# microscopic-image-analysis/geosss

Measured on AMD Instinct MI355X. Metric: mcmc_chain_steps_per_sec, higher is better.
Workload: dtype f64; 1 GPU; vmfmix_readme: shrinkage slice sampler, 1000000 chains/GPU x 1000 transitions per launch, thin=100; target=vmfmix_readme, d=3, chains_per_gpu=1000000, thin=100, mode=fast, kernel=screened_kernel<3, ScreenVmf<3, 3>>, kept_rows_layout=components, slice_steps=500, library_matches_tree=True, stream=philox-v3 (chain,step)-keyed; S2: tangent = one angle; 32-bit tries

## Files before the change

geosss_amd/csrc/gsss_device.h:

```cpp
#pragma once
#include <hip/hip_runtime.h>
#include <stdint.h>
#include <stdlib.h>

#include <algorithm>
#include <vector>

#include "../../include/gsss.h"
#include "gsss_counter_words.h"
#include "gsss_math.h"

namespace gsss {

constexpr int kBlock = 256;
constexpr double kTwoPi = 6.283185307179586;

struct TargetBlock {
    const double *blob;
    int32_t kind, d, k, dpad;
    double kappa;
    double scale;
};

struct RunBlock {
// ... 521 lines not shown
        hop = s[(size_t)r.r_hop * n];
        psum = s[(size_t)r.r_p * n];
        psq = s[(size_t)(r.r_p + 1) * n];
        pos = r.L > 0 ? (int)(cnt % (int64_t)r.L) : 0;
#pragma unroll
        for (int l = 0; l < kStatsMaxLags; ++l) {
            const bool in = l < r.L;
            lag[l] = in ? s[(size_t)(r.r_lag + (in ? l : 0)) * n] : 0.0;
            if (in) ring[(size_t)l * kBlock] = s[(size_t)(r.r_ring + l) * n];
        }
    }

    __device__ __forceinline__ void draw(const RunBlock &a, int64_t c, const double (&x)[D])
    {
        const size_t n = (size_t)a.n_chains;
        double *s = a.stats + c;
        const Rows r = rows(a);
        const double *w = a.stats_dirs, *h = a.stats_dirs + D, *modes = a.stats_dirs + 2 * D;
        double p = 0.0, xh = 0.0;
#pragma unroll
        for (int j = 0; j < D; ++j) {
            p = fma(x[j], w[j], p);
            xh = fma(x[j], h[j], xh);
        }
        if (cnt > 0) {
            double dot = 0.0, ph = 0.0;
#pragma unroll
            for (int j = 0; j < D; ++j) {
                dot = fma(prev[j], x[j], dot);
                ph = fma(prev[j], h[j], ph);
            }
            dist += acos(fmin(fmax(dot, -1.0), 1.0));
            const int sa = (xh > 0.0) - (xh < 0.0), sb = (ph > 0.0) - (ph < 0.0);
            if (sa != sb) hop += 1.0;
        }
        int t = 0;
#pragma unroll
        for (int i = 0; i < D; ++i) {
            prev[i] = x[i];
            sum[i] += x[i];
            if (r.second) {
#pragma unroll
                for (int j = i; j < D; ++j) {
                    if (kXXRegs)
                        xx[t] += x[i] * x[j];
                    else
                        s[(size_t)(r.r_xx + t) * n] += x[i] * x[j];
                    ++t;
                }
            }
        }
        if (r.K > 0) {
            int best = 0;
            double bv = -INFINITY;
            for (int k = 0; k < r.K; ++k) {
                double v = 0.0;
#pragma unroll
                for (int j = 0; j < D; ++j) v = fma(x[j], modes[k * D + j], v);
                if (v > bv) {
                    bv = v;
                    best = k;
                }
            }
            s[(size_t)(r.r_mode + best) * n] += 1.0;
        }
        psum += p;
        psq += p * p;
        if (r.L > 0) {
            const int lm = cnt < (int64_t)r.L ? (int)cnt : r.L;
            int si = pos;
#pragma unroll
            for (int l = 1; l <= kStatsMaxLags; ++l) {
                si = si == 0 ? r.L - 1 : si - 1;
                if (l <= lm) lag[l - 1] += p * ring[(size_t)si * kBlock];
            }
            ring[(size_t)pos * kBlock] = p;
            if (cnt < r.L) s[(size_t)(r.r_head + cnt) * n] = p;
            pos = pos + 1 == r.L ? 0 : pos + 1;
        }
        ++cnt;
    }

    __device__ __forceinline__ void store(const RunBlock &a, int64_t c)
    {
        const size_t n = (size_t)a.n_chains;
        double *s = a.stats + c;
        const Rows r = rows(a);
        s[0] = (double)cnt;
#pragma unroll
        for (int i = 0; i < D; ++i) {
            s[(size_t)(r.r_prev + i) * n] = prev[i];
            s[(size_t)(r.r_sum + i) * n] = sum[i];
        }
        if (kXXRegs && r.second) {
#pragma unroll
            for (int t = 0; t < kT; ++t) s[(size_t)(r.r_xx + t) * n] = xx[t];
        }
        s[(size_t)r.r_dist * n] = dist;
        s[(size_t)r.r_hop * n] = hop;
        s[(size_t)r.r_p * n] = psum;
        s[(size_t)(r.r_p + 1) * n] = psq;
#pragma unroll
        for (int l = 0; l < kStatsMaxLags; ++l) {
            if (l < r.L) {
                s[(size_t)(r.r_lag + l) * n] = lag[l];
                s[(size_t)(r.r_ring + l) * n] = ring[(size_t)l * kBlock];
            }
        }
    }
};

__device__ __forceinline__ void philox4x32_10(uint32_t c0, uint32_t c1, uint32_t c2, uint32_t c3, uint32_t k0,
                                              uint32_t k1, uint32_t (&o)[4])
{
    k0 = (uint32_t)__builtin_amdgcn_readfirstlane((int)k0);
    k1 = (uint32_t)__builtin_amdgcn_readfirstlane((int)k1);
    asm volatile("" : "+s"(k0), "+s"(k1));
#pragma unroll
    for (int r = 0; r < 10; ++r) {
        const uint64_t p0 = (uint64_t)0xD2511F53u * c0;
        const uint64_t p1 = (uint64_t)0xCD9E8D57u * c2;
        const uint32_t n0 = __builtin_amdgcn_bitop3_b32((uint32_t)(p1 >> 32), c1, k0, 0x96);
        const uint32_t n2 = __builtin_amdgcn_bitop3_b32((uint32_t)(p0 >> 32), c3, k1, 0x96);
        c1 = (uint32_t)p1;
        c3 = (uint32_t)p0;
        c0 = n0;
        c2 = n2;
        k0 += 0x9E3779B9u;
        k1 += 0xBB67AE85u;
    }
    o[0] = c0; o[1] = c1; o[2] = c2; o[3] = c3;
}

__device__ __forceinline__ double try_uniform(uint32_t w) { return (double)w * 0x1.0p-32; }

__device__ __forceinline__ double u53(uint32_t a, uint32_t b)
{
    return fma((double)(a >> 5), 67108864.0, (double)(b >> 6)) * 0x1.0p-53;
}

__device__ __forceinline__ void box_muller32(uint32_t wr, uint32_t wa, double &z0, double &z1)
{
    float f0, f1;
    fm::box_muller_f32(wr, wa, f0, f1);
    z0 = (double)f0;
    z1 = (double)f1;
}

__device__ __forceinline__ void box_muller32(uint32_t wr, uint32_t wa, const fm::Tables &, double &z0, double &z1)
{
    box_muller32(wr, wa, z0, z1);
}

__device__ __forceinline__ void tangent3(double n0, double n1, double n2, double sn, double cs, double &u0, double &u1, double &u2)
{
    const double s = copysign(1.0, n2);
    const double a = -1.0 / (s + n2);
    const double b = n0 * n1 * a;
    const double b10 = 1.0 + s * n0 * n0 * a, b11 = s * b, b12 = -s * n0;
    const double b20 = b, b21 = s + n1 * n1 * a, b22 = -n1;
    u0 = fma(sn, b20, cs * b10);
    u1 = fma(sn, b21, cs * b11);
    u2 = fma(sn, b22, cs * b12);
}

constexpr int kTabLds = 2 * 64 + 2;
__device__ __forceinline__ fm::Tables stage_tables(double *lds_after_params)
{
    double *buf = lds_after_params + ((reinterpret_cast<uintptr_t>(lds_after_params) >> 3) & 1u);
    for (int i = threadIdx.x; i < 64; i += kBlock) fm::table_entry(buf, i);
    return fm::Tables{buf, nullptr};
}

constexpr uint64_t kInitStep = 0xFFFFFFFFFFFFull;

template <int D_>
struct LaneVec {
    static constexpr int L = 1;
    static constexpr int N = D_;
    static constexpr int DPAD = D_;
    static constexpr bool kExactDim = true;
    __device__ static __forceinline__ int comp(int , int i) { return i; }
    __device__ static __forceinline__ double reduce(double v) { return v; }
};

constexpr int kDppXor1 = 0xB1;
constexpr int kDppXor2 = 0x4E;
constexpr int kDppHalfMirror = 0x141;
constexpr int kDppMirror = 0x140;

template <int CTRL>
__device__ __forceinline__ double dpp_move(double v)
{
    const int lo = __builtin_amdgcn_update_dpp(0, __double2loint(v), CTRL, 0xF, 0xF, true);
    const int hi = __builtin_amdgcn_update_dpp(0, __double2hiint(v), CTRL, 0xF, 0xF, true);
    return __hiloint2double(hi, lo);
}
template <int CTRL>
__device__ __forceinline__ int dpp_move(int v)
{
    return __builtin_amdgcn_update_dpp(0, v, CTRL, 0xF, 0xF, true);
}
__device__ __forceinline__ double lane_broadcast(double v, int lane)
{
    const int lo = __builtin_amdgcn_readlane(__double2loint(v), lane);
    const int hi = __builtin_amdgcn_readlane(__double2hiint(v), lane);
    return __hiloint2double(hi, lo);
}

template <int L_>
__device__ __forceinline__ double group_sum(double v)
{
    if (L_ >= 2) v += dpp_move<kDppXor1>(v);
    if (L_ >= 4) v += dpp_move<kDppXor2>(v);
    if (L_ >= 8) v += dpp_move<kDppHalfMirror>(v);
    if (L_ >= 16) v += dpp_move<kDppMirror>(v);
    if (L_ == 64) {
        const double r0 = lane_broadcast(v, 0), r1 = lane_broadcast(v, 16);
        const double r2 = lane_broadcast(v, 32), r3 = lane_broadcast(v, 48);
        v = (r0 + r1) + (r2 + r3);
    }
    return v;
}

template <int L_, int S_>
struct CoopVec {
    static_assert(S_ % 4 == 0, "slots come in quads");
    static constexpr int L = L_;
    static constexpr int N = S_;
    static constexpr int DPAD = L_ * S_;
    static constexpr bool kExactDim = false;
    __device__ static __forceinline__ int comp(int g, int i) { return 4 * (g + L_ * (i >> 2)) + (i & 3); }
    static_assert(L_ == 2 || L_ == 4 || L_ == 8 || L_ == 16 || L_ == 64, "group sizes with a DPP reduction");
    __device__ static __forceinline__ double reduce(double v) { return group_sum<L_>(v); }
};

template <class V>
__device__ __forceinline__ double vdot(const double (&a)[V::N], const double (&b)[V::N])
{
    double s = 0.0;
#pragma unroll
    for (int i = 0; i < V::N; ++i) s = fma(a[i], b[i], s);
    return V::reduce(s);
}

template <class V>
__device__ __forceinline__ void stats_update_group(const RunBlock &a, int64_t c, int g, int d, const double (&x)[V::N])
{
    constexpr int N = V::N, LG = V::L;
    const size_t n = (size_t)a.n_chains;
    double *s = a.stats + c;
    const int K = a.stats_modes, L = a.stats_lags;
    const bool second = !(a.stats_flags & GSSS_STATS_NO_SECOND_MOMENT);
    const int T = second ? d * (d + 1) / 2 : 0;
    const int r_prev = 1, r_sum = 1 + d, r_xx = 1 + 2 * d, r_dist = r_xx + T, r_hop = r_dist + 1, r_mode = r_hop + 1;
    const int r_p = r_mode + K, r_lag = r_p + 2, r_ring = r_lag + L, r_head = r_ring + L;
    const double *w = a.stats_dirs, *h = a.stats_dirs + d, *modes = a.stats_dirs + 2 * d;
    const int64_t cnt = (int64_t)V::reduce(g == 0 ? s[0] : 0.0);
    double p = 0.0, xh = 0.0, dot = 0.0, ph = 0.0;
#pragma unroll
    for (int i = 0; i < N; ++i) {
        const int cc = V::comp(g, i);
        if (cc < d) {
            p = fma(x[i], w[cc], p);
            xh = fma(x[i], h[cc], xh);
            if (cnt > 0) {
                const double pj = s[(size_t)(r_prev + cc) * n];
                dot = fma(pj, x[i], dot);
                ph = fma(pj, h[cc], ph);
            }
        }
    }
    p = V::reduce(p);
    xh = V::reduce(xh);
    dot = V::reduce(dot);
    ph = V::reduce(ph);
    if (cnt > 0 && g == 0) {
        s[(size_t)r_dist * n] += acos(fmin(fmax(dot, -1.0), 1.0));
        const int sa = (xh > 0.0) - (xh < 0.0), sb = (ph > 0.0) - (ph < 0.0);
        if (sa != sb) s[(size_t)r_hop * n] += 1.0;
    }
#pragma unroll
    for (int i = 0; i < N; ++i) {
        const int cc = V::comp(g, i);
        if (cc < d) {
            s[(size_t)(r_prev + cc) * n] = x[i];
            s[(size_t)(r_sum + cc) * n] += x[i];
        }
    }
    if (second) {
        const int base = (int)(threadIdx.x % 64) - g;
        for (int jl = 0; jl < LG; ++jl) {
#pragma unroll
            for (int j = 0; j < N; ++j) {
                const double xj = __shfl(x[j], base + jl);
                const int cj = V::comp(jl, j);
#pragma unroll
                for (int i = 0; i < N; ++i) {
                    const int ci = V::comp(g, i);
                    if (cj < d && ci <= cj) s[(size_t)(r_xx + ci * d - ci * (ci - 1) / 2 + (cj - ci)) * n] += x[i] * xj;
                }
            }
        }
    }
    if (K > 0) {
        int best = 0;
        double bv = -INFINITY;
        for (int k = 0; k < K; ++k) {
            double v = 0.0;
#pragma unroll
// ... 1106 lines not shown
```

geosss_amd/csrc/gsss_screen.h:

```cpp
#pragma once
#include <type_traits>

#include "gsss_fast.h"
#include "gsss_screen_consts.h"

namespace gsss {

enum : int32_t { kFinalAccept = 3, kFinalDecide = 4, kFinalInHi = 2 };
__device__ __forceinline__ bool is_final(int32_t st) { return st >= kFinalAccept; }
__device__ __forceinline__ bool is_decide(int32_t st) { return st == kFinalDecide || st == kFinalDecide + kFinalInHi; }

__device__ __forceinline__ void sincos_rev32(double theta, float &s, float &c)
{
    const float t = (float)(theta * 0.15915494309189535);
    s = __builtin_amdgcn_sinf(t);
    c = __builtin_amdgcn_cosf(t);
}

__device__ __forceinline__ float log2_32(double v)
{
    int e;
    const double m = frexp(v, &e);
    return (float)e + __builtin_amdgcn_logf((float)m);
}

template <int D, int KC>
struct ScreenVmf : FastVmf<D, KC> {
    using Base = FastVmf<D, KC>;
    using Coef = typename Base::Coef;
    static constexpr int kCoef32Floats = 3 * KC + 1;
    static constexpr int kParkSkip = KC >= 6 ? 2 * KC : 0;
    static constexpr int kMinWaves = D > 10 ? ((D <= 12 && KC <= 3) ? 3 : 2) : (KC >= 6 ? 3 : ((D == 3 && KC <= 3) ? 5 : 1));
    static constexpr int kTradeMin = KC >= 6 ? 24 : 1;
    static constexpr int kSharedMinWaves = kMinWaves;
    static constexpr bool kCompact = false;
    static constexpr bool kOneAhead = KC == 10 || (KC == 6 && D <= 8) || (KC == 16 && D <= 5) || (KC == 4 && D == 3) || (KC == 3 && D == 4);
    static constexpr bool kStageRows = kOneAhead;
    static constexpr bool kHoldRows = false;
    static constexpr bool kPreferOne = kOneAhead;
    static constexpr int kNumpyWaves = (KC >= 10 || (D >= 9 && KC >= 6)) ? 2 : ((D <= 4 && KC <= 3) ? 4 : 3);
    static constexpr bool kRegenThr = D == 3 && KC <= 3;
    static constexpr bool kLog2Rows = D == 3 && KC <= 3;
    static_assert(!kLog2Rows || kParkSkip == 0, "refill() would have to form its floats from the scaled rows too");
    __host__ __device__ static constexpr size_t log2_doubles() { return kLog2Rows ? (size_t)KC * D + KC : 0; }
    __device__ void stage_log2(double *lds, const TargetBlock &tb)
    {
        constexpr double L = 1.4426950408889634074;
        Base::stage(lds, tb);
        __syncthreads();
        const int rows = (int)Base::lds_doubles();
        for (int i = threadIdx.x; i < rows; i += kBlock) lds[rows + i] = lds[i] * L;
    }
    __device__ __forceinline__ static void dots(const double *rows, int k, const double (&x)[D], const double (&u)[D], double &ax, double &au)
    {
        ax = 0.0, au = 0.0;
#pragma unroll
        for (int j = 0; j < D; ++j) {
            const double mkj = rows[k * D + j];
            ax = fma(mkj, x[j], ax);
            au = fma(mkj, u[j], au);
        }
    }
    __device__ __forceinline__ void retail(float (&)[kCoef32Floats]) const {}
    __device__ __forceinline__ void refill(const double (&x)[D], const double (&u)[D], float (&q)[kCoef32Floats]) const
    {
        constexpr double L = 1.4426950408889634074;
#pragma unroll
        for (int k = 0; k < KC; ++k) {
            double ax = 0.0, au = 0.0;
#pragma unroll
            for (int j = 0; j < D; ++j) {
                const double mkj = this->mu[k * D + j];
                ax = fma(mkj, x[j], ax);
                au = fma(mkj, u[j], au);
            }
            q[k] = (float)(ax * L);
            q[KC + k] = (float)(au * L);
        }
    }

    __device__ __forceinline__ void coeffs(Coef &cf, const double (&x)[D], const double (&u)[D]) const
    {
#pragma unroll
        for (int k = 0; k < KC; ++k) dots(this->mu, k, x, u, cf.ax[k], cf.au[k]);
        double m = -INFINITY;
#pragma unroll
        for (int k = 0; k < KC; ++k) m = fmax(m, cf.ax[k] + this->logc[k]);
        cf.m = m;
    }
    __device__ __forceinline__ bool make32(const Coef &cf, double u_thr, float (&q)[kCoef32Floats]) const
    {
        constexpr double L = 1.4426950408889634074;
        float s0 = 0.0f;
#pragma unroll
        for (int k = 0; k < KC; ++k) {
            q[k] = (float)(cf.ax[k] * L);
            q[KC + k] = (float)(cf.au[k] * L);
            q[2 * KC + k] = (float)((this->logc[k] - cf.m) * L);
            s0 += __builtin_amdgcn_exp2f(q[k] + q[2 * KC + k]);
        }
        return finish32(u_thr, q, s0);
    }
    __device__ __forceinline__ bool finish32(double u_thr, float (&q)[kCoef32Floats], float s0) const
    {
        float b = 0.0f;
        int e;
        const float m0 = frexpf(s0, &e);
        const float t2 = ((float)e + __builtin_amdgcn_logf(m0)) + log2_32(u_thr);
#pragma unroll
        for (int k = 0; k < KC; ++k) {
            q[2 * KC + k] -= t2;
            if (k < this->K) b = fmaxf(b, fabsf(q[k]) + fabsf(q[KC + k]) + fabsf(q[2 * KC + k]));
        }
        b += fabsf(t2);
        const float e_a = b * (kSinCosErr32 + 7.0f * kUnit32) + (1.4427f * (kExp2Err32 + (float)KC * kUnit32) + 6.0e-8f + kLog2Err32);
        float margin = 1.25f * (0.69315f * e_a * (1.0f + e_a) + kExp2Err32 + (float)KC * kUnit32) + 1.0e-7f;
        if (!(u_thr > 1e-290) || !(margin < 0.25f)) margin = INFINITY;
        q[3 * KC] = margin;
        return s0 > 0.5f && s0 < 3.0e38f;
    }
    __device__ __forceinline__ double threshold(Coef &cf, const double (&x)[D], const double (&u)[D], double u_thr) const
    {
        return this->make(cf, x, u, 0.0, true) * u_thr;
    }
    __device__ __forceinline__ int screen(const float (&q)[kCoef32Floats], float c, float s) const
    {
        typedef float f2 __attribute__((ext_vector_type(2)));
        const f2 c2 = {c, c}, s2 = {s, s};
        float sum;
        constexpr int kPacked = KC >= 6 ? KC - KC % 2 : 0;
#pragma unroll
        for (int k = 0; k + 1 < kPacked + 1 && k < kPacked; k += 2) {
            const f2 ax = {q[k], q[k + 1]}, au = {q[KC + k], q[KC + k + 1]}, lc = {q[2 * KC + k], q[2 * KC + k + 1]};
            const f2 e = __builtin_elementwise_fma(c2, ax, __builtin_elementwise_fma(s2, au, lc));
            sum = k == 0 ? __builtin_amdgcn_exp2f(e.x) : sum + __builtin_amdgcn_exp2f(e.x);
            sum += __builtin_amdgcn_exp2f(e.y);
        }
#pragma unroll
        for (int k = kPacked; k < KC; ++k) {
            const float t = __builtin_amdgcn_exp2f(fmaf(c, q[k], fmaf(s, q[KC + k], q[2 * KC + k])));
            sum = k == 0 ? t : sum + t;
        }
        const float margin = q[3 * KC], dev = sum - 1.0f;
        return dev < -margin ? -1 : (dev > margin ? 1 : 0);
    }
    __device__ __forceinline__ double level_exact(const Coef &cf, double c, double s) const
    {
        double a[KC];
#pragma unroll
        for (int k = 0; k < KC; ++k) a[k] = fma(c, cf.ax[k], fma(s, cf.au[k], this->logc[k])) - cf.m;
        return this->level_full(a);
    }
    __device__ __forceinline__ bool setup32(const double (&x)[D], const double (&u)[D], double u_thr, float (&q)[kCoef32Floats]) const
    {
        Coef cf;
        coeffs(cf, x, u);
        return make32(cf, u_thr, q);
    }
    __device__ __forceinline__ bool setup32_log2(const double (&x)[D], const double (&u)[D], double u_thr, float (&q)[kCoef32Floats]) const
    {
        const double *mul = this->mu + Base::lds_doubles(), *lcl = this->logc + Base::lds_doubles();
        double m = -INFINITY;
        float s0 = 0.0f;
#pragma unroll
        for (int k = 0; k < KC; ++k) {
            double ax, au;
            dots(mul, k, x, u, ax, au);
            q[k] = (float)ax;
            q[KC + k] = (float)au;
            m = fmax(m, ax + lcl[k]);
        }
#pragma unroll
        for (int k = 0; k < KC; ++k) {
            q[2 * KC + k] = (float)(lcl[k] - m);
            s0 += __builtin_amdgcn_exp2f(q[k] + q[2 * KC + k]);
        }
        return finish32(u_thr, q, s0);
    }
    __device__ __forceinline__ bool decide(const double (&x)[D], const double (&u)[D], double u_thr, double c, double s) const
    {
        Coef cf;
        const double thr = threshold(cf, x, u, u_thr);
        return level_exact(cf, c, s) > thr;
    }
};

template <class TP, class = void>
struct screen_log2_rows : std::false_type {};
template <class TP>
struct screen_log2_rows<TP, std::enable_if_t<TP::kLog2Rows>> : std::true_type {};
template <class TP>
__host__ __device__ constexpr size_t screen_row_doubles()
{
    if constexpr (screen_log2_rows<TP>::value)
        return TP::lds_doubles() + TP::log2_doubles();
    else
        return TP::lds_doubles();
}

template <int D>
struct ScreenBingham : FastBingham<D> {
    using Base = FastBingham<D>;
    using Coef = typename Base::Coef;
    static constexpr int kCoef32Floats = 6;
    static constexpr int kParkSkip = 0, kMinWaves = D > 10 ? 2 : 1, kTradeMin = 1;
    static constexpr int kSharedMinWaves = kMinWaves;
    static constexpr bool kCompact = false, kRegenThr = false, kStageRows = true;
    static constexpr bool kPreferOne = D != 6;
    static constexpr bool kHoldRows = true;
    static constexpr int kNumpyWaves = D >= 7 ? 2 : 3;
    __device__ __forceinline__ void retail(float (&)[kCoef32Floats]) const {}
    __device__ __forceinline__ void refill(const double (&)[D], const double (&)[D], float (&)[kCoef32Floats]) const {}
    __device__ __forceinline__ void coeffs(Coef &cf, const double (&x)[D], const double (&u)[D]) const
    {
        (void)this->make(cf, x, u, 0.0, true);
    }
    __device__ __forceinline__ bool make32(const Coef &cf, double u_thr, float (&q)[kCoef32Floats]) const
    {
        const double lvl0 = cf.qxx + cf.bx;
        const float l2 = log2_32(u_thr);
        const float lu = l2 * 0.69314718f;
        q[0] = (float)(cf.qxx - lvl0) - lu;
        q[1] = (float)cf.qxu;
        q[2] = (float)(cf.quu - lvl0) - lu;
        q[3] = (float)cf.bx;
        q[4] = (float)cf.bu;
        const float sum = fabsf(q[0]) + fabsf(q[1]) + fabsf(q[2]) + fabsf(q[3]) + fabsf(q[4]);
        const float e_lu = (kLog2Err32 + 2.0f * kUnit32 * fabsf(l2)) * 0.6932f + kUnit32 * (fabsf(lu) + fabsf(q[0]) + fabsf(q[2]));
        float margin = 1.25f * (sum * (2.0f * kSinCosErr32 + 6.0f * kUnit32) + e_lu) + 1.0e-30f;
        if (!(u_thr > 1e-290) || !(margin < 1.0e30f)) margin = INFINITY;
        q[5] = margin;
        return lvl0 > -INFINITY && lvl0 < INFINITY;
    }
    __device__ __forceinline__ int screen(const float (&q)[kCoef32Floats], float c, float s) const
    {
        const float g = fmaf(c, fmaf(c, q[0], fmaf(s, q[1], q[3])), s * fmaf(s, q[2], q[4]));
        return g < -q[5] ? -1 : (g > q[5] ? 1 : 0);
    }
    __device__ __forceinline__ double threshold(Coef &cf, const double (&x)[D], const double (&u)[D], double u_thr) const
    {
        return this->make(cf, x, u, 0.0, true) + fm::log_fast(u_thr);
    }
    __device__ __forceinline__ double level_exact(const Coef &cf, double c, double s) const { return this->level(cf, c, s); }
    __device__ __forceinline__ bool setup32(const double (&x)[D], const double (&u)[D], double u_thr, float (&q)[kCoef32Floats]) const
    {
        Coef cf;
        coeffs(cf, x, u);
        return make32(cf, u_thr, q);
    }
    __device__ __forceinline__ bool decide(const double (&x)[D], const double (&u)[D], double u_thr, double c, double s) const
    {
        Coef cf;
        const double thr = threshold(cf, x, u, u_thr);
        return level_exact(cf, c, s) > thr;
    }
};

template <int D>
struct ScreenBinghamDiag {
    static constexpr bool kLinear = false;
    static constexpr int kCoef32Floats = 4;
    static constexpr int kParkSkip = 0, kMinWaves = D >= 14 ? 2 : (D >= 9 ? 3 : 1), kTradeMin = 1;
    static constexpr int kSharedMinWaves = D == 13 ? 2 : kMinWaves;
    static constexpr bool kCompact = true, kRegenThr = true, kStageRows = true;
    static constexpr bool kPreferOne = D >= 5;
    static constexpr bool kHoldRows = true;
    static constexpr int kNumpyWaves = 3;
    const double *a;
    struct Coef {
        double qxx, qxu, quu;
    };
    __host__ __device__ static constexpr size_t lds_doubles() { return (size_t)D; }
    __device__ void stage(double *lds, const TargetBlock &tb)
    {
        for (int i = threadIdx.x; i < D; i += kBlock) lds[i] = tb.blob[(size_t)i * D + i];
        a = lds;
    }
    __device__ static double staged(const double *blob, int , int i) { return blob[(size_t)i * D + i]; }
    __device__ __forceinline__ void attach(const double *rows, const TargetBlock &) { a = rows; }
    __device__ __forceinline__ double make(Coef &cf, const double (&x)[D], const double (&u)[D]) const
    {
        double qxx = 0.0, qxu = 0.0, quu = 0.0;
#pragma unroll
        for (int j = 0; j < D; ++j) {
            const double ajj = a[j];
            const double xa = x[j] * ajj, ua = u[j] * ajj;
            qxx = fma(xa, x[j], qxx);
            qxu = fma(xa, u[j], fma(ua, x[j], qxu));
            quu = fma(ua, u[j], quu);
        }
        cf.qxx = qxx;
        cf.qxu = qxu;
        cf.quu = quu;
        return qxx + 0.0;
    }
    __device__ __forceinline__ double level_exact(const Coef &cf, double c, double s) const
    {
        return fma(c * c, cf.qxx, fma(c * s, cf.qxu, (s * s) * cf.quu)) + fma(c, 0.0, s * 0.0);
    }
    __device__ __forceinline__ void retail(float (&q)[kCoef32Floats]) const
    {
        const float sum = fabsf(q[0]) + fabsf(q[1]) + fabsf(q[2]);
        const float l2 = 1.4428f * fabsf(q[0]);
        const float e_lu = (kLog2Err32 + 2.0f * kUnit32 * l2) * 0.6932f + kUnit32 * (2.0f * fabsf(q[0]) + fabsf(q[2]));
        float margin = 1.25f * (sum * (2.0f * kSinCosErr32 + 6.0f * kUnit32) + e_lu) + 1.0e-30f;
        if (!(margin < 1.0e30f)) margin = INFINITY;
        q[3] = margin;
    }
    __device__ __forceinline__ void refill(const double (&)[D], const double (&)[D], float (&)[kCoef32Floats]) const {}
    __device__ __forceinline__ bool setup32(const double (&x)[D], const double (&u)[D], double u_thr, float (&q)[kCoef32Floats]) const
    {
        Coef cf;
        const double lvl0 = make(cf, x, u);
        const float lu = log2_32(u_thr) * 0.69314718f;
        q[0] = 0.0f - lu;
        q[1] = (float)cf.qxu;
        q[2] = (float)(cf.quu - lvl0) - lu;
        if (!(u_thr > 1e-290)) q[0] = INFINITY;
        retail(q);
        return lvl0 > -INFINITY && lvl0 < INFINITY;
    }
    __device__ __forceinline__ int screen(const float (&q)[kCoef32Floats], float c, float s) const
    {
// ... 423 lines not shown
    const int32_t id1 = a.one_per_lane ? n : id0 + kBlock;

    Chain cur;
    int32_t slot = 0;
    int32_t parked_status = kDone;
    StatsLane<D> sl;
    const bool stats_onchip = STATS && a.stats_onchip > 0;

    constexpr bool kLean = !BATCH && lean_words<TP>::value;
    auto chain_id = [&]() { return slot ? id1 : id0; };
    auto philox = [&]() {
        PhiloxDraws<V, true> dr;
        dr.tab = tab;
        if constexpr (kLean) {
            dr.init_step(a, chain_id(), cur.steps_done, D);
        } else {
            dr.init(a, chain_id(), D);
            dr.begin_step(a.step_offset + (uint64_t)cur.steps_done);
        }
        return dr;
    };
    auto replay_take = [&]() -> double {
        if constexpr (NUMPY) return nd.next_double();
        if (cur.cursor >= (int32_t)a.replay_stride) {
            cur.err |= GSSS_CHAIN_REPLAY_EXHAUSTED;
            return 0.5;
        }
        return a.replay[(size_t)chain_id() * a.replay_stride + cur.cursor++];
    };
    auto count_tries = [&]() { gsss::count_tries(cur); };
    auto needs_service = [](int32_t st) { return st == kPending || is_final(st); };

    auto init = [&]() {
        const int32_t c = chain_id();
        const bool valid = c < n;
        const int32_t cc = valid ? c : 0;
#pragma unroll
        for (int j = 0; j < D; ++j) cur.x[j] = a.state[(size_t)j * n + cc];
#pragma unroll
        for (int j = 0; j < D; ++j) cur.u[j] = 0.0;
#pragma unroll
        for (int i = 0; i < Chain::kQ; ++i) cur.q[i] = 0.0f;
        cur.lo = cur.hi = cur.thr = 0.0;
        cur.n_try = 0u;
        cur.steps_done = s_begin;
        cur.row = s_begin / thin;
        cur.err = 0;
        cur.cursor = 0;
        cur.t = 0;
        cur.status = (valid && n_steps > s_begin) ? kPending : kDone;
        if constexpr (NUMPY) nd.init(a, cc, D);
        if constexpr (STATS) {
            if (stats_onchip && valid) sl.load(a, cc, reinterpret_cast<double *>(park));
        }
        if (sliced && valid) {
            if (SliceSched::dead(a, a.one_per_lane ? kBlock : kChunk)[cc] != 0) cur.status = kDone;
            if (timed_out && cur.status != kDone) {
                cur.err |= GSSS_CHAIN_MAX_TRIES | GSSS_CHAIN_COUNTER_SATURATED;
                cur.status = kDone;
            }
        }
    };

    auto setup = [&]() {
        double u_thr, u_th0;
        uint32_t w_phi = 0u;
        if (REPLAY) {
            if constexpr (NUMPY) {
#pragma unroll
                for (int j = 0; j < D; ++j) cur.u[j] = nd.standard_normal();
            } else if (cur.cursor + D <= (int32_t)a.replay_stride) {
#pragma unroll
                for (int j = 0; j < D; ++j)
                    cur.u[j] = a.replay[(size_t)chain_id() * a.replay_stride + cur.cursor + j];
                cur.cursor += D;
            } else {
#pragma unroll
                for (int j = 0; j < D; ++j) cur.u[j] = 0.5;
                cur.cursor = (int32_t)a.replay_stride;
                cur.err |= GSSS_CHAIN_REPLAY_EXHAUSTED;
            }
            u_thr = replay_take();
            u_th0 = shrink ? replay_take() : 0.0;
        } else {
            const PhiloxDraws<V, true> dr = philox();
            if constexpr (D == 3) {
                dr.step_s2(u_thr, u_th0, w_phi);
            } else {
                dr.normals(cur.u, 0);
                dr.block(0u, u_thr, u_th0);
            }
        }
        bool x_ok;
        if constexpr (D == 3 && !REPLAY) {
            const double xx = vdot<V>(cur.x, cur.x);
            x_ok = xx < INFINITY;
            const double rnx = inv_norm(xx);
            const double nrm[3] = {cur.x[0] * rnx, cur.x[1] * rnx, cur.x[2] * rnx};
            philox().tangent(nrm, cur.u, 0, w_phi);
        } else
        {
            const double xx = vdot<V>(cur.x, cur.x);
            x_ok = xx < INFINITY;
            const double rnx = inv_norm(xx);
            double cz = 0.0;
#pragma unroll
            for (int j = 0; j < D; ++j) cz = fma(cur.u[j], cur.x[j] * rnx, cz);
#pragma unroll
            for (int j = 0; j < D; ++j) cur.u[j] = fma(-cz, cur.x[j] * rnx, cur.u[j]);
            const double rnw = inv_norm(vdot<V>(cur.u, cur.u));
#pragma unroll
            for (int j = 0; j < D; ++j) cur.u[j] *= rnw;
        }
        cur.thr = u_thr;
        bool finite;
        if constexpr (kLog2)
            finite = tp.setup32_log2(cur.x, cur.u, u_thr, reinterpret_cast<float (&)[TP::kCoef32Floats]>(cur.q));
        else
            finite = tp.setup32(cur.x, cur.u, u_thr, reinterpret_cast<float (&)[TP::kCoef32Floats]>(cur.q));
        if constexpr (D > 10) {
            if (a.screen == 2) cur.q[TP::kCoef32Floats - 1] = INFINITY;
        }
        if (shrink) {
            cur.hi = kTwoPi * u_th0;
            cur.lo = cur.hi - kTwoPi;
        } else {
            cur.lo = 0.0;
            cur.hi = kTwoPi;
        }
        cur.t = 0;
        cur.status = kReady;
        if (!finite || !x_ok) {
            cur.err |= GSSS_CHAIN_NONFINITE;
            cur.status = kDone;
        }
    };

    constexpr bool kTry32 = !REPLAY;
    constexpr int kPerAttempt = kTry32 ? 4 : 2;
    auto attempt = [&]() {
        if (cur.t >= max_tries) {
            count_tries();
            cur.err |= GSSS_CHAIN_MAX_TRIES;
            cur.status = kDone;
            return;
        }
        double u_pair[2];
        uint32_t w_try[4];
        if constexpr (kTry32) {
            philox().words(kTryBase + (uint32_t)(cur.t >> 2), w_try);
        } else if (!REPLAY) {
            philox().block(kTryBase + (uint32_t)(cur.t >> 1), u_pair[0], u_pair[1]);
        }
        const int first = REPLAY ? 0 : (cur.t & (kPerAttempt - 1));
        const int lim = first + (max_tries - cur.t);
        bool stopped = false;
#pragma unroll
        for (int h = 0; h < kPerAttempt; ++h) {
            if (!stopped && h >= first && h < lim &&
                !(REPLAY && (cur.err & GSSS_CHAIN_REPLAY_EXHAUSTED))) {
                double uu;
                if constexpr (kTry32)
                    uu = try_uniform(w_try[h]);
                else
                    uu = REPLAY ? replay_take() : u_pair[h & 1];
                if (REPLAY && (cur.err & GSSS_CHAIN_REPLAY_EXHAUSTED)) {
                    stopped = true;
                } else {
                    const double theta = fma(cur.hi - cur.lo, uu, cur.lo);
                    ++cur.t;
                    float s32, c32;
                    sincos_rev32(theta, s32, c32);
                    const int verdict = tp.screen(reinterpret_cast<const float (&)[TP::kCoef32Floats]>(cur.q), c32, s32);
                    const bool rej = verdict < 0, neg = theta < 0.0, moves = !rej | shrink;
                    cur.lo = (moves & neg) ? theta : cur.lo;
                    cur.hi = (moves & !neg) ? theta : cur.hi;
                    cur.status = rej ? cur.status : ((verdict > 0 ? kFinalAccept : kFinalDecide) + (neg ? 0 : kFinalInHi));
                    stopped = !rej;
                }
            }
        }
        if (REPLAY && (cur.err & GSSS_CHAIN_REPLAY_EXHAUSTED) && cur.status == kReady) {
            count_tries();
            cur.status = kDone;
        }
    };

    auto unstage = [&](double *p_next) {
#pragma unroll
        for (int b = 0; b < kStageP - 1; ++b) {
            if (b < n_staged) {
                double *q = p_next - (size_t)(n_staged - b) * D;
#pragma unroll
                for (int j = 0; j < D; ++j) q[j] = stage[(size_t)(b * D + j) * kBlock];
            }
        }
        n_staged = 0;
    };
    auto finalise = [&]() {
        const double theta = cur.status >= kFinalAccept + kFinalInHi ? cur.hi : cur.lo;
        double sn, cs;
        fm::sincos_tab(theta, tab, sn, cs);
        bool accepted = true;
        if (is_decide(cur.status)) {
            double u_thr = cur.thr;
            if constexpr (Chain::kRegenThr && !REPLAY) {
                double u_th0;
                if constexpr (D == 3) {
                    uint32_t w_phi;
                    philox().step_s2(u_thr, u_th0, w_phi);
                } else {
                    philox().block(0u, u_thr, u_th0);
                }
            }
            accepted = tp.decide(cur.x, cur.u, u_thr, cs, sn);
        }
        if (accepted) {
#pragma unroll
            for (int j = 0; j < D; ++j) cur.x[j] = fma(sn, cur.u[j], cs * cur.x[j]);
            count_tries();
            ++cur.steps_done;
            bool keep = false;
            if (a.samples != nullptr || STATS) {
                if constexpr (Chain::kCompact) {
                    int32_t rows;
                    keep = divides(cur.steps_done, thin, rcp_thin, rows);
                    cur.row = rows - 1;
                } else {
                    keep = cur.steps_done == (cur.row + 1) * thin;
                }
            }
            if (keep) {
                if (a.samples != nullptr) {
                    if (kStageP > 1 && a.stage_rows) {
                        double *p = &a.samples[sample_index(a, cur.row, 0, D, chain_id())];
                        const bool ends_on_sector = (reinterpret_cast<uintptr_t>(p + D) & 31u) == 0u;
                        if (!ends_on_sector && n_staged < kStageP - 1) {
#pragma unroll
                            for (int j = 0; j < D; ++j) stage[(size_t)(n_staged * D + j) * kBlock] = cur.x[j];
                            ++n_staged;
                        } else {
                            unstage(p);
#pragma unroll
                            for (int j = 0; j < D; ++j) p[j] = cur.x[j];
                        }
                    } else if constexpr (kLean) {
                        const KeptRow kr = kept_row(a, cur.row, D, chain_id());
#pragma unroll
                        for (int j = 0; j < D; ++j) kr.p[(int64_t)j * kr.step] = cur.x[j];
                    } else {
#pragma unroll
                        for (int j = 0; j < D; ++j) a.samples[sample_index(a, cur.row, j, D, chain_id())] = cur.x[j];
                    }
                }
                if constexpr (STATS) {
                    if (stats_onchip)
                        sl.draw(a, chain_id(), cur.x);
                    else
                        stats_update<D>(a, chain_id(), cur.x);
                }
                ++cur.row;
            }
            const bool exhausted = REPLAY && (cur.err & GSSS_CHAIN_REPLAY_EXHAUSTED);
            cur.status = (cur.steps_done < n_steps && !exhausted) ? kPending : kDone;
        } else {
            if (!shrink) cur.hi = kTwoPi;
            cur.status = kReady;
        }
    };

    auto pack_flags = [&]() { return cur.t | (cur.status << 25) | (int32_t)((uint32_t)cur.err << 28); };
    auto trade = [&]() {
        unsigned long long *p = park;
        auto word = [&](double &v) {
            lds_trade(v, p);
            p += kBlock;
        };
#pragma unroll
        for (int j = 0; j < D; ++j) word(cur.x[j]);
#pragma unroll
        for (int j = 0; j < D; ++j) word(cur.u[j]);
        word(cur.lo);
        word(cur.hi);
        if constexpr (Chain::kCompact) {
            if (REPLAY) word(cur.thr);
            lds_trade<kLean>(cur.q[0], cur.q[1], p);
            p += kBlock;
            lds_trade<kLean>(cur.q[2], cur.steps_done, p);
            p += kBlock;
        } else {
            if (!Chain::kRegenThr || REPLAY) word(cur.thr);
#pragma unroll
            for (int i = Chain::kSkip; i < Chain::kQ; i += 2) {
                lds_trade<kLean>(cur.q[i], cur.q[i + 1], p);
                p += kBlock;
            }
            lds_trade<kLean>(cur.steps_done, cur.row, p);
            p += kBlock;
        }
        if (REPLAY) {
            int32_t zero = 0;
            lds_trade<kLean>(cur.cursor, zero, p);
            p += kBlock;
        }
        const int32_t st = cur.status;
        int32_t nt = (int32_t)cur.n_try, packed = pack_flags();
        lds_trade<kLean>(nt, packed, p);
        cur.n_try = (uint32_t)nt;
        cur.t = packed & 0x1FFFFFF;
        cur.status = (packed >> 25) & 7;
        cur.err = (int32_t)((uint32_t)packed >> 28);
        parked_status = st;
        slot ^= 1;
        if (Chain::kSkip > 0 && (cur.status == kReady || is_decide(cur.status))) tp.refill(cur.x, cur.u, reinterpret_cast<float (&)[TP::kCoef32Floats]>(cur.q));
        if constexpr (Chain::kCompact) tp.retail(reinterpret_cast<float (&)[TP::kCoef32Floats]>(cur.q));
    };

    constexpr bool kThrough = !STATS;
    auto put_out = [&](auto *p, auto v) {
        if (kThrough && sliced)
            SliceSched::hand_over(p, v);
        else
            *p = v;
    };
    auto flush = [&]() {
        const int32_t c = chain_id();
        if (c >= n) return;
        if (kStageP > 1 && n_staged > 0) unstage(&a.samples[sample_index(a, cur.steps_done / thin, 0, D, c)]);
        if constexpr (NUMPY) nd.finish(a, c, true);
        if constexpr (STATS) {
            if (stats_onchip) sl.store(a, c);
        }
#pragma unroll
// ... 228 lines not shown
```

geosss_amd/csrc/gsss_verify.hip:

```cpp
#include <hip/hip_runtime.h>
#include <math.h>
#include <stdint.h>
#include <string.h>

#include "../../include/gsss.h"
#include "gsss_device.h"
#include "gsss_screen_consts.h"

namespace gsss {
namespace {

constexpr int kSweepOut = 4;

__device__ void atomic_max_double(double *p, double v)
{
    unsigned long long *u = reinterpret_cast<unsigned long long *>(p);
    unsigned long long old = *u;
    while (__longlong_as_double((long long)old) < v) {
        const unsigned long long seen = atomicCAS(u, old, (unsigned long long)__double_as_longlong(v));
        if (seen == old) break;
        old = seen;
    }
}

__device__ __forceinline__ double half_ulp(float x)
{
    int e;
    (void)frexpf(fabsf(x), &e);
    if (e < -125) e = -125;
    return ldexp(1.0, e - 25);
}

__global__ void __launch_bounds__(kBlock) f32_sweep_kernel(uint32_t lo_bits, uint64_t count, int which, double *acc)
{
    double e[kSweepOut] = {0.0, 0.0, 0.0, 0.0};
    const double two_pi = 6.283185307179586476925286766559, inv_ln2 = 1.4426950408889634;
    for (uint64_t i = (uint64_t)blockIdx.x * blockDim.x + threadIdx.x; i < count; i += (uint64_t)gridDim.x * blockDim.x) {
        const float x = __uint_as_float(lo_bits + (uint32_t)i);
        if (which == 0) {
            const double a = two_pi * (double)x, slack = two_pi * (fabsf(x) == 1.0f ? 2.9802322387695312e-8 : half_ulp(x));
            const double es = fabs((double)__builtin_amdgcn_sinf(x) - sin(a)), ec = fabs((double)__builtin_amdgcn_cosf(x) - cos(a));
            e[0] = fmax(e[0], es);
            e[1] = fmax(e[1], ec);
            e[2] = fmax(e[2], es + slack);
            e[3] = fmax(e[3], ec + slack);
        } else if (which == 1) {
            const double want = exp2((double)x), got = (double)__builtin_amdgcn_exp2f(x);
            if (want >= 3.4028235677973366e38) e[2] += (got == (double)INFINITY) ? 0.0 : 1.0;
            else if (want >= 1.1754943508222875e-38) e[0] = fmax(e[0], fabs(got - want) / want);
            else e[1] = fmax(e[1], fabs(got - want));
        } else if (which == 2) {
            const double err = fabs((double)__builtin_amdgcn_logf(x) - log2((double)x));
            e[0] = fmax(e[0], err);
            if (x <= 1.0f) e[1] = fmax(e[1], err + half_ulp(x) * inv_ln2 / ((double)x - half_ulp(x)));
        } else {
            const double want = sqrt((double)x);
            e[0] = fmax(e[0], fabs((double)__builtin_amdgcn_sqrtf(x) - want) / want);
        }
    }
    for (int k = 0; k < kSweepOut; ++k) {
        if (which == 1 && k == 2) {
            if (e[k] > 0.0) atomicAdd(&acc[k], e[k]);
        } else if (e[k] > 0.0) {
            atomic_max_double(&acc[k], e[k]);
        }
    }
}

struct Range {
    float a, b;
};

}
}

extern "C" {

int gsss_screen_constants(double *out, int32_t n)
{
    using namespace gsss;
    if (!out || n < 5) {
        set_error("gsss_screen_constants needs room for 5 doubles");
        return GSSS_E_INVALID;
    }
    out[0] = (double)kSinCosErr32;
    out[1] = (double)kExp2Err32;
    out[2] = (double)kLog2Err32;
    out[3] = (double)kSqrtRelErr32;
    out[4] = (double)kUnit32;
    return GSSS_OK;
}

int gsss_f32_error_sweep(int32_t which, double *out_host, uint64_t *n_swept_out, int device, void *stream)
{
    using namespace gsss;
    if (which < 0 || which > 3 || !out_host) {
        set_error("bad argument to gsss_f32_error_sweep");
        return GSSS_E_INVALID;
    }
    int prev = 0;
    if (hipGetDevice(&prev) != hipSuccess || hipSetDevice(device) != hipSuccess) {
        set_error("gsss_f32_error_sweep: no such device");
        return GSSS_E_HIP;
    }
    static const Range ranges[4][2] = {{{0.0f, 1.0f}, {-0.0f, -1.0f}},
                                       {{0.0f, 3.4028234664e38f}, {-0.0f, -3.4028234664e38f}},
                                       {{0.5f, 2.0f}, {1.0f, 1.0f}},
                                       {{1.17549435e-38f, 3.4028234664e38f}, {1.0f, 1.0f}}};
    hipStream_t st = static_cast<hipStream_t>(stream);
    double *acc = nullptr;
    int rc = GSSS_OK;
    uint64_t swept = 0;
    double zero[kSweepOut] = {0.0, 0.0, 0.0, 0.0};
    if (hipMalloc(&acc, sizeof(zero)) != hipSuccess || hipMemcpyAsync(acc, zero, sizeof(zero), hipMemcpyHostToDevice, st) != hipSuccess) {
        rc = GSSS_E_HIP;
    } else {
        for (int r = 0; r < 2 && rc == GSSS_OK; ++r) {
            if (r == 1 && which >= 2) break;
            uint32_t ua, ub;
            memcpy(&ua, &ranges[which][r].a, 4);
            memcpy(&ub, &ranges[which][r].b, 4);
            const uint64_t count = (uint64_t)(ub - ua) + 1;
            rc = launch_kernel("f32 sweep", f32_sweep_kernel, 16384, 0, st, nullptr, ua, count, (int)which, acc);
            swept += count;
        }
        if (rc == GSSS_OK && (hipMemcpyAsync(out_host, acc, sizeof(zero), hipMemcpyDeviceToHost, st) != hipSuccess ||
                              hipStreamSynchronize(st) != hipSuccess))
            rc = GSSS_E_HIP;
    }
    if (acc) (void)hipFree(acc);
    (void)hipSetDevice(prev);
    if (rc != GSSS_OK) {
        (void)hipGetLastError();
        set_error("gsss_f32_error_sweep: a HIP call failed");
        return rc;
    }
    if (n_swept_out) *n_swept_out = swept;
    return GSSS_OK;
}

}
```

Measured before the change: 53.35 billion chain-steps/s.

## Use range-limited reciprocal in tangent3 and restructure lean 32-bit try loop

Replaces the IEEE double divide in tangent3 with an rcp seed plus Newton refinements and a final correction. The denominator s+n2 lies in [1,2] in magnitude, so no special-case handling is needed. A device sweep checks that the result is bit-identical to the true divide. The lean 32-bit try path now shifts the Philox words to the front (only when some lane in the wavefront is misaligned) and writes the chain status once after the loop instead of on every try. It also seeds the log2 max from the first component rather than -inf. Together these aim to cut divide latency and per-try select and predicate overhead, at the cost of extra code complexity and a wavefront ballot.

```diff
diff --git a/geosss_amd/csrc/gsss_device.h b/geosss_amd/csrc/gsss_device.h
--- a/geosss_amd/csrc/gsss_device.h
+++ b/geosss_amd/csrc/gsss_device.h
@@ -697,10 +697,19 @@
     box_muller32(wr, wa, z0, z1);
 }
 
+__device__ __forceinline__ double neg_recip_unit_range(double d)
+{
+    const double r0 = __builtin_amdgcn_rcp(d);
+    const double r1 = fma(r0, fma(-d, r0, 1.0), r0);
+    const double r2 = fma(r1, fma(-d, r1, 1.0), r1);
+    const double q = -1.0 * r2;
+    return fma(fma(-d, q, -1.0), r2, q);
+}
+
 __device__ __forceinline__ void tangent3(double n0, double n1, double n2, double sn, double cs, double &u0, double &u1, double &u2)
 {
     const double s = copysign(1.0, n2);
-    const double a = -1.0 / (s + n2);
+    const double a = neg_recip_unit_range(s + n2);
     const double b = n0 * n1 * a;
     const double b10 = 1.0 + s * n0 * n0 * a, b11 = s * b, b12 = -s * n0;
     const double b20 = b, b21 = s + n1 * n1 * a, b22 = -n1;
diff --git a/geosss_amd/csrc/gsss_screen.h b/geosss_amd/csrc/gsss_screen.h
--- a/geosss_amd/csrc/gsss_screen.h
+++ b/geosss_amd/csrc/gsss_screen.h
@@ -160,7 +160,7 @@
     __device__ __forceinline__ bool setup32_log2(const double (&x)[D], const double (&u)[D], double u_thr, float (&q)[kCoef32Floats]) const
     {
         const double *mul = this->mu + Base::lds_doubles(), *lcl = this->logc + Base::lds_doubles();
-        double m = -INFINITY;
+        double m = 0.0;
         float s0 = 0.0f;
 #pragma unroll
         for (int k = 0; k < KC; ++k) {
@@ -168,7 +168,7 @@
             dots(mul, k, x, u, ax, au);
             q[k] = (float)ax;
             q[KC + k] = (float)au;
-            m = fmax(m, ax + lcl[k]);
+            m = k == 0 ? ax + lcl[k] : fmax(m, ax + lcl[k]);
         }
 #pragma unroll
         for (int k = 0; k < KC; ++k) {
@@ -898,12 +898,25 @@
         } else if (!REPLAY) {
             philox().block(kTryBase + (uint32_t)(cur.t >> 1), u_pair[0], u_pair[1]);
         }
-        const int first = REPLAY ? 0 : (cur.t & (kPerAttempt - 1));
-        const int lim = first + (max_tries - cur.t);
+        [[maybe_unused]] int first = REPLAY ? 0 : (cur.t & (kPerAttempt - 1));
+        int cnt = first + (max_tries - cur.t);
+        constexpr bool kLeanTry = kLean && kTry32;
+        if constexpr (kLeanTry) {
+            cnt = max_tries - cur.t;
+            if (__ballot(first != 0) != 0ull) {
+                const bool r1 = (first & 1) != 0, r2 = (first & 2) != 0;
+                const uint32_t a0 = r1 ? w_try[1] : w_try[0], a1 = r1 ? w_try[2] : w_try[1], a2 = r1 ? w_try[3] : w_try[2];
+                w_try[0] = r2 ? a2 : a0;
+                w_try[1] = r2 ? w_try[3] : a1;
+                w_try[2] = a2;
+                cnt = min(cnt, kPerAttempt - first);
+            }
+        }
         bool stopped = false;
+        [[maybe_unused]] bool stop_accept = false, stop_in_hi = false;
 #pragma unroll
         for (int h = 0; h < kPerAttempt; ++h) {
-            if (!stopped && h >= first && h < lim &&
+            if (!stopped && (kLeanTry || h >= first) && h < cnt &&
                 !(REPLAY && (cur.err & GSSS_CHAIN_REPLAY_EXHAUSTED))) {
                 double uu;
                 if constexpr (kTry32)
@@ -921,10 +934,18 @@
                     const bool rej = verdict < 0, neg = theta < 0.0, moves = !rej | shrink;
                     cur.lo = (moves & neg) ? theta : cur.lo;
                     cur.hi = (moves & !neg) ? theta : cur.hi;
-                    cur.status = rej ? cur.status : ((verdict > 0 ? kFinalAccept : kFinalDecide) + (neg ? 0 : kFinalInHi));
+                    if constexpr (kLeanTry) {
+                        stop_accept = verdict > 0;
+                        stop_in_hi = !neg;
+                    } else {
+                        cur.status = rej ? cur.status : ((verdict > 0 ? kFinalAccept : kFinalDecide) + (neg ? 0 : kFinalInHi));
+                    }
                     stopped = !rej;
                 }
             }
+        }
+        if constexpr (kLeanTry) {
+            if (stopped) cur.status = (stop_accept ? kFinalAccept : kFinalDecide) + (stop_in_hi ? kFinalInHi : 0);
         }
         if (REPLAY && (cur.err & GSSS_CHAIN_REPLAY_EXHAUSTED) && cur.status == kReady) {
             count_tries();
diff --git a/geosss_amd/csrc/gsss_verify.hip b/geosss_amd/csrc/gsss_verify.hip
--- a/geosss_amd/csrc/gsss_verify.hip
+++ b/geosss_amd/csrc/gsss_verify.hip
@@ -67,6 +67,28 @@
     }
 }
 
+constexpr uint64_t kDivSweep = 1ull << 22;
+__global__ void __launch_bounds__(kBlock) div_sweep_kernel(uint64_t count, double *acc)
+{
+    const double special[14] = {0.0, -0.0, 1.0, -1.0, 0x1.fffffffffffffp-1, -0x1.fffffffffffffp-1, 0x1.0000000000001p+0,
+                                -0x1.0000000000001p+0, 0x1.0p-1074, -0x1.0p-1074, 0x1.0p-1022, -0x1.0p-1022, 0x1.0p-53, -0x1.0p-53};
+    double differ = 0.0, outside = 0.0;
+    for (uint64_t i = (uint64_t)blockIdx.x * blockDim.x + threadIdx.x; i < count; i += (uint64_t)gridDim.x * blockDim.x) {
+        uint64_t z = (i + 1) * 0x9E3779B97F4A7C15ull;
+        z = (z ^ (z >> 30)) * 0xBF58476D1CE4E5B9ull;
+        z = (z ^ (z >> 27)) * 0x94D049BB133111EBull;
+        z ^= z >> 31;
+        double n2 = fma((double)(z >> 11) * 0x1.0p-53, 0x1.0p-21, -1.0 + (double)i * 0x1.0p-21);
+        if (i < 14) n2 = special[i];
+        const double d = copysign(1.0, n2) + n2;
+        const double want = -1.0 / d, got = neg_recip_unit_range(d);
+        differ += __double_as_longlong(want) != __double_as_longlong(got) ? 1.0 : 0.0;
+        outside += (fabs(d) >= 1.0 && fabs(d) <= 2.0) ? 0.0 : 1.0;
+    }
+    if (differ > 0.0) atomicAdd(&acc[0], differ);
+    if (outside > 0.0) atomicAdd(&acc[1], outside);
+}
+
 struct Range {
     float a, b;
 };
@@ -94,7 +116,7 @@
 int gsss_f32_error_sweep(int32_t which, double *out_host, uint64_t *n_swept_out, int device, void *stream)
 {
     using namespace gsss;
-    if (which < 0 || which > 3 || !out_host) {
+    if (which < 0 || which > 4 || !out_host) {
         set_error("bad argument to gsss_f32_error_sweep");
         return GSSS_E_INVALID;
     }
@@ -115,7 +137,11 @@
     if (hipMalloc(&acc, sizeof(zero)) != hipSuccess || hipMemcpyAsync(acc, zero, sizeof(zero), hipMemcpyHostToDevice, st) != hipSuccess) {
         rc = GSSS_E_HIP;
     } else {
-        for (int r = 0; r < 2 && rc == GSSS_OK; ++r) {
+        if (which == 4) {
+            rc = launch_kernel("divide sweep", div_sweep_kernel, 1024, 0, st, nullptr, kDivSweep, acc);
+            swept = kDivSweep;
+        }
+        for (int r = 0; r < 2 && rc == GSSS_OK && which < 4; ++r) {
             if (r == 1 && which >= 2) break;
             uint32_t ua, ub;
             memcpy(&ua, &ranges[which][r].a, 4);
```

Result: slower. 52.32 billion chain-steps/s (-1.9%).
